# angela000/DQNFlappyBird

Hardware: AMD Instinct MI355X
Metric: env steps/sec (whole node) + DQN grad-steps/sec, 80x80x4 batch=32 (higher is better)
Workload: dtype f32

## Files before the change

dqnflappybird_amd/csrc/fb_qnet.hip:

```cpp
#include <math.h>
#include <stdlib.h>
#include "fb_common.h"

#ifndef FK_ABL
#define FK_ABL 0
#endif
#ifndef BW_ABL
#define BW_ABL 0
#endif

namespace {

typedef float f32x16 __attribute__((ext_vector_type(16)));

constexpr int OFF_W1 = 0, OFF_B1 = 8192, OFF_W2 = 8224, OFF_B2 = 40992, OFF_W3 = 41056, OFF_B3 = 77920,
              OFF_WF1 = 77984;
constexpr int CONV_PARAMS = OFF_WF1;
#include "fb_head.h"
#include "fb_sampler.h"
#include "fb_gather.h"
constexpr int MAXTB = 256;


struct Slice { const float *params; const uint8_t *states; int s_off, count; const uint16_t *w1s; int fshift; };
// ... 13 lines not shown
#pragma unroll
        for (int r = 0; r < 16; r++) { const int row = base + drow(r, lane); if (row < limit) body(r, row); }
    }
}

template <int NW, class F>
__device__ __forceinline__ void reduce_rows(const f32x16 &acc, float *red, int wave, int lane, int base, int limit, F body) {
    if (wave < NW) {
#pragma unroll
        for (int r = 0; r < 16; r++) red[(wave * 16 + r) * 64 + lane] = acc[r];
    }
    __syncthreads();
    if (wave >= 8) return;
    float v[2];
#pragma unroll
    for (int q = 0; q < 2; q++) {
        const int r = 2 * wave + q;
        v[q] = red[r * 64 + lane];
#pragma unroll
        for (int w = 1; w < NW; w++) v[q] += red[(w * 16 + r) * 64 + lane];
    }
    if (base + 32 <= limit) {
#pragma unroll
        for (int q = 0; q < 2; q++) body(v[q], 2 * wave + q, base + drow(2 * wave + q, lane));
    } else {
#pragma unroll
        for (int q = 0; q < 2; q++) { const int row = base + drow(2 * wave + q, lane); if (row < limit) body(v[q], 2 * wave + q, row); }
    }
}

__device__ __forceinline__ void keep(float &x) { asm volatile("" : "+v"(x)); }
__device__ __forceinline__ float rbf(float x, bool rb) { return rb ? (float)(__bf16)x : x; }
__device__ __forceinline__ void keep(int &x) { asm volatile("" : "+v"(x)); }

typedef __bf16 bf16x8 __attribute__((ext_vector_type(8)));

__device__ __forceinline__ uint32_t f32_to_bf16_rn(float x) {
    const uint32_t u = __float_as_uint(x);
    return (u + 0x7FFFu + ((u >> 16) & 1u)) >> 16;
}

__device__ __forceinline__ void split3(float x, uint32_t &hi, uint32_t &mid, uint32_t &lo) {
    hi = f32_to_bf16_rn(x);
    const float r1 = x - __uint_as_float(hi << 16);
    mid = f32_to_bf16_rn(r1);
    lo = f32_to_bf16_rn(r1 - __uint_as_float(mid << 16));
}

typedef __bf16 bf16x2 __attribute__((ext_vector_type(2)));
typedef float f32x2 __attribute__((ext_vector_type(2)));
__device__ __forceinline__ void split3x2(float x0, float x1, uint32_t &hi, uint32_t &mid, uint32_t &lo) {
    const f32x2 x = {x0, x1};
    const bf16x2 h = __builtin_convertvector(x, bf16x2);
    const f32x2 r1 = x - __builtin_convertvector(h, f32x2);
    const bf16x2 m = __builtin_convertvector(r1, bf16x2);
    const f32x2 r2 = r1 - __builtin_convertvector(m, f32x2);
    const bf16x2 l = __builtin_convertvector(r2, bf16x2);
    hi = __builtin_bit_cast(uint32_t, h); mid = __builtin_bit_cast(uint32_t, m); lo = __builtin_bit_cast(uint32_t, l);
}

typedef _Float16 f16x8 __attribute__((ext_vector_type(8)));
typedef _Float16 f16x2 __attribute__((ext_vector_type(2)));
constexpr float F16_LO_SCALE = 4096.f, F16_LO_UNSCALE = 1.f / 4096.f;
__device__ __forceinline__ void split2x2(float x0, float x1, uint32_t &hi, uint32_t &lo) {
    const f32x2 x = {x0, x1};
    const f16x2 h = __builtin_convertvector(x, f16x2);
// ... 1647 lines not shown
    float nq[AT], mean = 0.f;
#pragma unroll
    for (int a = 0; a < AT; a++) {
        const int o = (a < A ? a : 0) * N + il;
        nq[a] = draw(LQ.eout + o) * (ns[a] + H.sig[H.off.bq + o]);
        if (a < A) mean += nq[a];
    }
    if (DUEL) {
        mean /= (float)A;
        const float vn = draw(LV.eout + il) * (nv + H.sig[H.off.bv + il]);
#pragma unroll
        for (int a = 0; a < AT; a++) lg[a] += (vn + nq[a]) - mean;
    } else {
#pragma unroll
        for (int a = 0; a < AT; a++) lg[a] += nq[a];
    }
    float qv[AT];
    const float z = H.sup.vmin + (float)(on ? lane : 0) * H.sup.dz;
    c51_q<AT>(lg, on, z, qv);
    if (lane == 0 && live) {
#pragma unroll
        for (int a = 0; a < AT; a++) if (a < A) H.q[(size_t)smp * A + a] = qv[a];
        int best = 0;
#pragma unroll
        for (int a = 1; a < AT; a++) if (a < A && qv[a] > qv[best]) best = a;
        const fb_u4 o = fb_philox(H.seed_lo, H.seed_hi, (uint32_t)key, H.step_lo, H.stream, H.step_hi);
        const float u = (float)(o.x >> 8) * (1.0f / 16777216.0f);
        if (u <= H.epsilon) best = (int)(((unsigned long long)o.y * (unsigned)A) >> 32);
        H.actions[smp] = (uint8_t)best;
    }
}

typedef float f32x4 __attribute__((ext_vector_type(4)));
struct FkArgs { Slices sl; const float *h3; float *hf; float *qpart; int FC, A, dueling, stot; NetOff off; };
constexpr int FK_ROW = 204;

__global__ __launch_bounds__(512) void fc1_fk_kernel(FkArgs a) {
    __shared__ float ast[8 * 16 * FK_ROW];
    __shared__ float red[8 * 4 * 64];
    const Slice s = a.sl.s[blockIdx.z];
    const int M = s.count, m0 = blockIdx.x * 16, n0 = blockIdx.y * 16;
    if (m0 >= M) return;
    const int lane = threadIdx.x & 63, wave = threadIdx.x >> 6, r = lane & 15, g = lane >> 4;
    const int kw = wave * 200;
    const float *bcol = s.params + OFF_WF1 + (size_t)(kw + 50 * g) * a.FC + n0 + r;
    float bv[50];
#pragma unroll
    for (int t = 0; t < 50; t++) bv[t] = bcol[(size_t)(FK_ABL == 2 ? 0 : t) * a.FC];
    float hb = s.params[a.off.bf1 + n0 + r], hw[MAXA + 1];
#pragma unroll
    for (int c = 0; c < MAXA; c++) hw[c] = s.params[a.off.wq + (n0 + r) * a.A + (c < a.A ? c : 0)];
    hw[MAXA] = s.params[(a.dueling ? a.off.wv : a.off.bf1) + n0 + r];
    float *mine = ast + wave * 16 * FK_ROW;
    float4 st[13];
#pragma unroll
    for (int i = 0; i < 13; i++) {
        const int idx = lane + 64 * i, row = idx < 800 ? idx / 50 : 0, c4 = idx < 800 ? idx - row * 50 : 0;
        const int mr = m0 + row < M ? m0 + row : M - 1;
        st[i] = *reinterpret_cast<const float4 *>(a.h3 + (size_t)(s.s_off + mr) * 1600 + kw + 4 * (FK_ABL == 3 ? 0 : c4));
    }
#pragma unroll
    for (int i = 0; i < 13; i++) {
        const int idx = lane + 64 * i, row = idx / 50, c4 = idx - row * 50;
        if (idx < 800) *reinterpret_cast<float4 *>(mine + row * FK_ROW + 4 * c4) = st[i];
    }
    __builtin_amdgcn_wave_barrier();
    asm volatile("s_waitcnt lgkmcnt(0)" ::: "memory");
    const float *arow = mine + r * FK_ROW + 50 * g;
    f32x4 acc0 = {0.f, 0.f, 0.f, 0.f}, acc1 = {0.f, 0.f, 0.f, 0.f};
    float2 av[25];
#pragma unroll
    for (int t = 0; t < 25; t++) av[t] = *reinterpret_cast<const float2 *>(arow + 2 * t);
#pragma unroll
    for (int t = 0; t < 25; t++) { keep(av[t].x); keep(av[t].y); }
#pragma unroll
    for (int t = 0; t < (FK_ABL == 1 ? 1 : 25); t++) {
        acc0 = __builtin_amdgcn_mfma_f32_16x16x4f32(rbf(av[t].x, a.sl.rb), rbf(bv[2 * t], a.sl.rb), acc0, 0, 0, 0);
        acc1 = __builtin_amdgcn_mfma_f32_16x16x4f32(rbf(av[t].y, a.sl.rb), rbf(bv[2 * t + 1], a.sl.rb), acc1, 0, 0, 0);
    }
#pragma unroll
    for (int q = 0; q < 4; q++) red[(wave * 4 + q) * 64 + lane] = acc0[q] + acc1[q];
    __syncthreads();
    if (threadIdx.x >= 256) return;
    const int reg = threadIdx.x >> 6, row = 4 * g + reg, col = r, mr = m0 + row, unit = n0 + col;
    float v = red[reg * 64 + lane];
#pragma unroll
    for (int w = 1; w < 8; w++) v += red[(w * 4 + reg) * 64 + lane];
    const bool live = mr < M;
    const size_t srow = (size_t)s.s_off + (live ? mr : M - 1);
    if (live) a.hf[srow * a.FC + unit] = v;
    if (!a.qpart || FK_ABL == 4) return;
    const float h = fmaxf(v + hb, 0.f);
    const int qs = a.A + 1;
    float *qo = a.qpart + (srow * (size_t)gridDim.y + blockIdx.y) * qs;
#pragma unroll
    for (int c = 0; c <= MAXA; c++) {
        if (c < a.A || (c == a.A && a.dueling)) {
            float x = h * (c == a.A ? hw[MAXA] : hw[c]);
#pragma unroll
            for (int o = 8; o > 0; o >>= 1) x += __shfl_xor(x, o, 16);
            if (col == 0 && live) qo[c] = x;
        }
    }
}

struct Bw1Args {
    int algo, B, FC, A, dueling, stot, n_dx, rb;
    NetOff off;
    const float *params, *pnext, *ptarget;
    const float *hf, *qpart, *h3;
    const uint8_t *act; const float *rew; const uint8_t *term; const float *isw;
    double gamma;
    float *grad, *dh3, *loss, *abs_err, *y_out;
    AdamDev *adam; int tick;
    FbGate gate;
};
constexpr int BW_DX_ROW = 4;
constexpr int BW_DW_ROW = 36;

template <int AT, bool DX>
__device__ __forceinline__ void fc1_bwd2_body(const Bw1Args &L, float *smem) {
    const int tid = threadIdx.x, lane = tid & 63, wave = tid >> 6, B = L.B, FC = L.FC, A = AT == MAXA ? L.A : AT;
    const float *P = L.params;
    float (*dadv)[MAXA] = reinterpret_cast<float (*)[MAXA]>(smem);
    float *dv = smem + MAXTB * MAXA, *lterm = dv + MAXTB, *dadv2 = lterm + MAXTB, *big = dadv2 + 2 * MAXTB;
    const bool lead = blockIdx.x == 0;
    const bool dbl = L.algo == FB_ALGO_DOUBLE;
    const int qs = A + 1, ntile = FC >> 4;
    constexpr bool dx_role = DX;
    const int mt = dx_role ? blockIdx.x / 50 : 0, t2 = dx_role ? 0 : blockIdx.x - L.n_dx, nt = t2 / 7, kg = t2 - nt * 7;
    const int kt = dx_role ? blockIdx.x - mt * 50 : kg * 8 + wave;
    auto unit_params = [&](int n, float &bias, float (&wq)[AT], float &wv) {
        bias = P[L.off.bf1 + n];
        wv = P[(L.dueling ? L.off.wv : L.off.bf1) + n];
#pragma unroll
        for (int c = 0; c < AT; c++) wq[c] = P[L.off.wq + n * A + (c < A ? c : 0)];
    };
    float pre_hf[32], pre_bias, pre_wq[AT], pre_wv, pre_a[16];
    float4 pre_w[8];
    if constexpr (DX) {
        const int ch = FC < 512 ? FC : 512, n = tid < ch ? tid : 0;
#pragma unroll
        for (int q = 0; q < 32; q++) { const int bq_ = mt * 32 + q; pre_hf[q] = L.hf[(size_t)(bq_ < B ? bq_ : 0) * FC + n]; }
        unit_params(n, pre_bias, pre_wq, pre_wv);
        const int kh = ch / 16, nbeg = wave * (ch / 8) + (lane >> 5) * kh;
        const float *brun = P + OFF_WF1 + (size_t)(kt * 32 + (lane & 31)) * FC + nbeg;
#pragma unroll
        for (int q = 0; q < 8; q++) pre_w[q] = *reinterpret_cast<const float4 *>(brun + (4 * q < kh ? 4 * q : 0));
#pragma unroll
        for (int q = 0; q < 16; q++) pre_a[q] = 0.f;
#pragma unroll
        for (int q = 0; q < 2; q++) { const int mr = mt * 32 + drow(2 * (wave & 7) + q, lane); pre_a[q] = L.h3[(size_t)(mr < B ? mr : 0) * 1600 + kt * 32 + (lane & 31)]; }
    } else {
        const int c = tid & 31;
#pragma unroll
        for (int q = 0; q < 2; q++) { const int b = (tid >> 5) + 16 * q; pre_hf[q] = L.hf[(size_t)(b < B ? b : 0) * FC + nt * 32 + c]; }
#pragma unroll
        for (int q = 2; q < 32; q++) pre_hf[q] = 0.f;
        unit_params(nt * 32 + c, pre_bias, pre_wq, pre_wv);
        const int ktc = kt < 50 ? kt : 0;
#pragma unroll
        for (int t = 0; t < 16; t++) { const int b = 2 * t + (lane >> 5); pre_a[t] = L.h3[(size_t)(b < B ? b : 0) * 1600 + ktc * 32 + (lane & 31)]; }
#pragma unroll
        for (int q = 0; q < 8; q++) pre_w[q] = make_float4(0.f, 0.f, 0.f, 0.f);
    }
    float bqs[AT], bqn[AT], bq3[AT];
#pragma unroll
    for (int c = 0; c < AT; c++) { const int cc = c < A ? c : 0; bqs[c] = L.params[L.off.bq + cc]; bqn[c] = L.pnext[L.off.bq + cc]; bq3[c] = L.ptarget[L.off.bq + cc]; }
    const int bvo = L.dueling ? L.off.bv : L.off.bq;
    float bvs = L.params[bvo], bvn = L.pnext[bvo], bv3 = L.ptarget[bvo];
    for (int b0 = 0; b0 < (BW_ABL == 1 ? 0 : B); b0 += 32) {
        const int b = b0 + (tid >> 4), j = tid & 15, bc = b < B ? b : 0;
        float rf = L.rew[bc], isw = L.isw ? L.isw[bc] : 1.f;
        int termb = L.term[bc], a_b = L.act[bc];
        float x0[2][AT + 1], x1[2][AT + 1], x2[2][AT + 1];
#pragma unroll
        for (int u = 0; u < 2; u++) {
            const int tile = j + 16 * u, tc = tile < ntile ? tile : 0;
            const float *q0 = L.qpart + ((size_t)bc * ntile + tc) * qs;
            const size_t rs = (size_t)ntile * qs;
#pragma unroll
            for (int c = 0; c <= AT; c++) {
                const int cc = c < qs ? c : 0;
                x0[u][c] = q0[cc]; x1[u][c] = q0[(size_t)B * rs + cc]; x2[u][c] = q0[(size_t)(dbl ? 2 * B : 0) * rs + cc];
            }
        }
        keep(rf); keep(isw); keep(termb); keep(a_b);
        float qsv[AT + 1], qnv[AT + 1], q3v[AT + 1];
#pragma unroll
        for (int c = 0; c <= AT; c++) {
            keep(x0[0][c]); keep(x1[0][c]); keep(x2[0][c]); keep(x0[1][c]); keep(x1[1][c]); keep(x2[1][c]);
            const bool on = c < A || (c == A && L.dueling), on0 = on && j < ntile, on1 = on && j + 16 < ntile;
            qsv[c] = (on0 ? x0[0][c] : 0.f) + (on1 ? x0[1][c] : 0.f);
            qnv[c] = (on0 ? x1[0][c] : 0.f) + (on1 ? x1[1][c] : 0.f);
            q3v[c] = (on0 ? x2[0][c] : 0.f) + (on1 ? x2[1][c] : 0.f);
        }
        for (int tile = j + 32; tile < ntile; tile += 16) {
// ... 39 lines not shown
        if (L.algo != FB_ALGO_PER) isw = 1.f;
        const double rr = rf == 0.1f ? 0.1 : (double)rf;
        const double yd = termb ? rr : rr + L.gamma * (double)sel;
        const float y = (float)yd;
        float qe = qsv[0];
#pragma unroll
        for (int c = 1; c < AT; c++) qe = c == a_b ? qsv[c] : qe;
        const float d = y - qe;
        const float scale = L.algo == FB_ALGO_DQN ? 2.f : 2.f / (float)B;
        const float gq = -scale * isw * d;
        const bool pg = L.algo == FB_ALGO_PG;
        float pgp[AT], pgl;
        {
            float mx = qsv[0], se = 0.f;
#pragma unroll
            for (int c = 1; c < AT; c++) mx = c < A ? fmaxf(mx, qsv[c]) : mx;
#pragma unroll
            for (int c = 0; c < AT; c++) { pgp[c] = c < A ? expf(qsv[c] - mx) : 0.f; se += pgp[c]; }
#pragma unroll
            for (int c = 0; c < AT; c++) pgp[c] /= se;
            pgl = logf(se) - (qe - mx);
        }
        const float pgw = rf / (float)L.gamma;
        if (j == 0 && b < B) {
            lterm[b] = pg ? pgl * pgw : isw * d * d;
            if (lead && L.abs_err) L.abs_err[b] = fabsf(d);
            if (lead && L.y_out) L.y_out[b] = y;
            dv[b] = L.dueling && !pg ? gq : 0.f;
#pragma unroll
            for (int c = 0; c < AT; c++) dadv[b][c] = pg ? (pgp[c] - (c == a_b ? 1.f : 0.f)) * pgw : (c == a_b ? gq : 0.f) - (L.dueling ? gq / (float)A : 0.f);
            if (AT == 2) { dadv2[2 * b] = dadv[b][0]; dadv2[2 * b + 1] = dadv[b][1]; }
        }
    }
#pragma unroll
    for (int q = 0; q < 32; q++) keep(pre_hf[q]);
#pragma unroll
    for (int q = 0; q < 16; q++) keep(pre_a[q]);
#pragma unroll
    for (int q = 0; q < 8; q++) { keep(pre_w[q].x); keep(pre_w[q].y); keep(pre_w[q].z); keep(pre_w[q].w); }
    __syncthreads();
    if (lead && tid == 0) {
        float sum = 0.f;
        for (int b = 0; b < B; b++) sum += lterm[b];
        *L.loss = L.algo == FB_ALGO_DQN || L.algo == FB_ALGO_PG ? sum : sum / (float)B;
        if (L.tick && L.adam->ticks == L.adam->applies) {
            AdamDev &ad = *L.adam;
            ad.alpha = ad.lr * sqrtf(1.f - ad.b2pow) / (1.f - ad.b1pow);
            ad.b1pow *= ad.b1; ad.b2pow *= ad.b2;
            ad.ticks += 1;
        }
    }
    if (lead && tid >= 64 && tid < 64 + A) { const int c = tid - 64; float sum = 0.f; for (int b = 0; b < B; b++) sum += dadv[b][c]; L.grad[L.off.bq + c] = sum; }
    if (lead && tid == 128 && L.dueling) { float sum = 0.f; for (int b = 0; b < B; b++) sum += dv[b]; L.grad[L.off.bv] = sum; }
    auto dhf_of = [&](int b, float hfv, float bias, const float (&wq)[AT], float wv, float &hout) {
        const float v = hfv + bias;
        float d = L.dueling ? dv[b] * wv : 0.f;
#pragma unroll
        for (int c = 0; c < AT; c++) if (c < A) d = fmaf(dadv[b][c], wq[c], d);
        hout = fmaxf(v, 0.f);
        return v > 0.f ? d : 0.f;
    };
    const int hl = lane >> 5, i = lane & 31, jj = lane & 31;
    if constexpr (DX) {
        const int RS = 512 + BW_DX_ROW;
        float *dh = big, *red = big + 32 * RS;
        f32x16 acc = {0};
        for (int nc = 0; nc < FC; nc += 512) {
            const int ch = FC - nc < 512 ? FC - nc : 512;
            if (nc) {
                __syncthreads();
                const int n = nc + (tid < ch ? tid : 0);
#pragma unroll
                for (int q = 0; q < 32; q++) { const int bq_ = mt * 32 + q; pre_hf[q] = L.hf[(size_t)(bq_ < B ? bq_ : 0) * FC + n]; }
                unit_params(n, pre_bias, pre_wq, pre_wv);
                const int kh = ch / 16, nbeg = wave * (ch / 8) + hl * kh;
                const float *brun = P + OFF_WF1 + (size_t)(kt * 32 + jj) * FC + nc + nbeg;
#pragma unroll
                for (int q = 0; q < 8; q++) pre_w[q] = *reinterpret_cast<const float4 *>(brun + (4 * q < kh ? 4 * q : 0));
            }
            if (tid < ch && BW_ABL != 2) {
                if (AT == 2 && !L.dueling) {
                    float4 da[16];
#pragma unroll
                    for (int q = 0; q < 16; q++) da[q] = *reinterpret_cast<const float4 *>(dadv2 + 2 * (mt * 32 + 2 * q < MAXTB - 1 ? mt * 32 + 2 * q : 0));
                    float o[32];
#pragma unroll
                    for (int q = 0; q < 16; q++) {
                        const float v0 = pre_hf[2 * q] + pre_bias, v1 = pre_hf[2 * q + 1] + pre_bias;
                        const float d0 = fmaf(da[q].y, pre_wq[1], fmaf(da[q].x, pre_wq[0], 0.f)), d1 = fmaf(da[q].w, pre_wq[1], fmaf(da[q].z, pre_wq[0], 0.f));
                        o[2 * q] = (v0 > 0.f && mt * 32 + 2 * q < B) ? d0 : 0.f;
                        o[2 * q + 1] = (v1 > 0.f && mt * 32 + 2 * q + 1 < B) ? d1 : 0.f;
                    }
#pragma unroll
                    for (int q = 0; q < 32; q++) dh[q * RS + tid] = o[q];
                } else {
#pragma unroll
                    for (int q = 0; q < 32; q++) {
                        float hv;
                        dh[q * RS + tid] = mt * 32 + q < B ? dhf_of(mt * 32 + q, pre_hf[q], pre_bias, pre_wq, pre_wv, hv) : 0.f;
                    }
                }
            }
            __syncthreads();
            const int kh = ch / 16, nbeg = wave * (ch / 8) + hl * kh;
            const float *arun = dh + i * RS + nbeg;
            float4 xa[8];
#pragma unroll
            for (int q = 0; q < 8; q++) xa[q] = *reinterpret_cast<const float4 *>(arun + (4 * q < kh ? 4 * q : 0));
#pragma unroll
            for (int q = 0; q < 8; q++) { keep(xa[q].x); keep(xa[q].y); keep(xa[q].z); keep(xa[q].w); }
#pragma unroll
            for (int q = 0; q < 8; q++) {
                if (4 * q < kh && BW_ABL != 3) {
                    const float4 x = xa[q], w = pre_w[q];
                    const bool rb = L.rb;
                    acc = mfma(rbf(x.x, rb), rbf(w.x, rb), acc); acc = mfma(rbf(x.y, rb), rbf(w.y, rb), acc);
                    acc = mfma(rbf(x.z, rb), rbf(w.z, rb), acc); acc = mfma(rbf(x.w, rb), rbf(w.w, rb), acc);
                }
            }
        }
        reduce_rows<8>(acc, red, wave, lane, mt * 32, B, [&](float v, int r, int mr) {
            const size_t o = (size_t)mr * 1600 + kt * 32 + jj;
            L.dh3[o] = BW_ABL == 4 ? v : (((r & 1) ? pre_a[1] : pre_a[0]) > 0.f ? v : 0.f);
        });
        return;
    }
    if (BW_ABL == 5) return;
    float *dh = big, *hh = big + MAXTB * BW_DW_ROW;
    {
        const int c = tid & 31;
#pragma unroll
        for (int q = 0; q < 2; q++) {
            const int b = (tid >> 5) + 16 * q;
// ... 1078 lines not shown
                (i >= off.bf1 && i < off.bf1 + FC) || (i >= off.bq && i < off.bq + A) || (dueling && i == off.bv);
    if (bias) { p[i] = 0.01f; return; }
    for (uint32_t ctr = 0;; ctr++) {
        const fb_u4 r = fb_philox(seed_lo, seed_hi, (uint32_t)i, ctr, FB_STREAM_INIT, 0u);
        const float u1 = ((r.x >> 8) + 1) * (1.0f / 16777216.0f), u2 = (r.y >> 8) * (1.0f / 16777216.0f);
        const float z = sqrtf(-2.f * logf(u1)) * cosf(6.28318530717958647692f * u2);
        if (fabsf(z) <= 2.f) { p[i] = 0.01f * z; return; }
    }
}

}

#ifndef FB_ADAM_GRID
#define FB_ADAM_GRID 1024
#endif
constexpr int ADAM_GRID = FB_ADAM_GRID;

struct fb_qnet {
    int arch, FC, A, max_batch;
    long long n;
    NetOff off;
    float *params[2], *adam_m, *adam_v, *grad, *slabs;
    float *slabs1;
    uint16_t *w1s[2];
    uint4 *wsp[2];
    uint16_t *zeros;
    uint16_t *a1s, *a3s;
    int nsplit;
    int nsplit_train;
    bool adam_ticked;
    AdamDev *adam;
    float *p1, *h2, *h3, *hf, *q;
    float *qpart;
    unsigned long long *ring_fo;
    hipEvent_t grad_ev;
    hipEvent_t grad_ev_recorded;
    uint8_t *amax;
    float *dhf, *dh3, *dh2, *dp1;
    float *gmax;
    int zmax;
    float *hf_act, *hp_act;
    FbSplitCtx *split;
    C51Sup sup;
    float kappa;
    float *c51_dl, *c51_xs, *c51_lt;
    NetOff hoff;
    float *heff[2];
    bool noisy;
    long long ntot;
    NoisyNet nnet;
    float *mst[2], *nz[2];
    int act_noise;
    float *nz_zero, *ht;
    uint4 *wsig;
    uint16_t *a3n;
    int *sig_seen;
    bool split_adam_pending;
};

static NetOff make_off(int FC, int A, int dueling) {
    NetOff o;
    o.bf1 = OFF_WF1 + 1600 * FC;
    int p = o.bf1 + FC;
    if (dueling) { o.wv = p; o.bv = p + FC; p = o.bv + 1; } else { o.wv = 0; o.bv = 0; }
    o.wq = p; o.bq = p + FC * A; o.n = o.bq + A;
    return o;
// ... 118 lines not shown
    h->hoff = is_c51d(h) ? make_off(fc_width, n_actions * sup.N, 0) : h->off;
    h->n = h->off.n;
    h->noisy = sigma0 >= 0.f;
    h->ntot = h->noisy ? 2 * h->n - OFF_WF1 : h->n;
    if (h->noisy) h->nnet = make_noisy(h->off, arch, fc_width, n_actions, sup.N, sigma0);
    h->zmax = 64;
    const size_t S = (size_t)3 * max_batch, nb = sizeof(float) * (size_t)h->n, nbt = sizeof(float) * (size_t)h->ntot;
    hipError_t e = hipSuccess;
    auto alloc = [&](void **p, size_t bytes) { if (e == hipSuccess) e = hipMalloc(p, bytes); if (e == hipSuccess) e = hipMemset(*p, 0, bytes); };
    alloc((void **)&h->params[0], nb); alloc((void **)&h->params[1], nb);
    alloc((void **)&h->adam_m, nbt); alloc((void **)&h->adam_v, nbt); alloc((void **)&h->grad, nbt);
    if (h->noisy) for (int w = 0; w < 2; w++) { alloc((void **)&h->mst[w], nbt); alloc((void **)&h->nz[w], sizeof(float) * (size_t)h->nnet.nz); }
    if (h->noisy) {
        alloc((void **)&h->nz_zero, sizeof(float) * (size_t)h->nnet.nz);
        alloc((void **)&h->wsig, sizeof(uint4) * (size_t)wsp_w3t(fc_width));
        alloc((void **)&h->a3n, S * 1600 * 6 + 256);
        alloc((void **)&h->ht, S * fc_width * 4 * FC1_SP_KS);
        alloc((void **)&h->sig_seen, sizeof(int));
        if (e == hipSuccess) e = hipMemset(h->sig_seen, 0xff, sizeof(int));
    }
    alloc((void **)&h->slabs, sizeof(float) * (size_t)h->zmax * CONV_PARAMS);
    if (2 * max_batch > h->zmax) alloc((void **)&h->slabs1, sizeof(float) * (size_t)2 * (max_batch < MAXTB ? max_batch : MAXTB) * CONV1_PARAMS);
    alloc((void **)&h->adam, sizeof(AdamDev));
    alloc((void **)&h->w1s[0], 3 * 8192 * 2); alloc((void **)&h->w1s[1], 3 * 8192 * 2);
    const size_t wsp_bytes = (size_t)wsp_total(fc_width) * sizeof(uint4);
    alloc((void **)&h->wsp[0], wsp_bytes); alloc((void **)&h->wsp[1], wsp_bytes);
    h->nsplit = 3; h->nsplit_train = 3;
    alloc((void **)&h->zeros, 256);
    alloc((void **)&h->a1s, S * 3200 * 6); alloc((void **)&h->a3s, S * 1600 * 6 + 256);
    alloc((void **)&h->p1, S * 3200 * 4); alloc((void **)&h->amax, S * 3200);
    alloc((void **)&h->h2, S * 1600 * 4); alloc((void **)&h->h3, S * 1600 * 4);
    alloc((void **)&h->hf, S * fc_width * 4 * FC1_KS); alloc((void **)&h->q, S * MAXA * 4);
    alloc((void **)&h->qpart, (size_t)(fc_width / 16) * S * (MAXA + 1) * 4);
    alloc((void **)&h->ring_fo, (size_t)max_batch * 4 * sizeof(unsigned long long));
    const size_t Bm = max_batch;
    alloc((void **)&h->dhf, Bm * fc_width * 4); alloc((void **)&h->dh3, Bm * 1600 * 4);
    alloc((void **)&h->dh2, Bm * 1600 * 4); alloc((void **)&h->dp1, Bm * 3200 * 4);
    alloc((void **)&h->gmax, (size_t)(fc_width / 16) * 4);
    alloc((void **)&h->hf_act, S * fc_width * 4 * FC1_SP_KS); alloc((void **)&h->hp_act, sizeof(float) * (size_t)(h->n - h->off.bf1));
    if (sup.N) { alloc((void **)&h->c51_dl, Bm * 64 * 4); alloc((void **)&h->c51_xs, Bm * fc_width * 4); alloc((void **)&h->c51_lt, Bm * 4); }
    if (is_c51d(h)) for (int w = 0; w < 2; w++) alloc((void **)&h->heff[w], sizeof(float) * (size_t)(h->hoff.n - h->off.bf1));
    if (e != hipSuccess) {
        fb_set_error(e == hipErrorOutOfMemory ? FB_ERR_NOMEM : FB_ERR_HIP, "fb_qnet_create: %s", hipGetErrorString(e));
        fb_qnet_destroy(h);
        return e == hipErrorOutOfMemory ? FB_ERR_NOMEM : FB_ERR_HIP;
    }
    *out = h;
    {
        AdamDev a; memset(&a, 0, sizeof(a));
        a.pver[0] = a.pver[1] = 1;
        if (hipMemcpy(h->adam, &a, sizeof(a), hipMemcpyHostToDevice) != hipSuccess) { fb_qnet_destroy(h); *out = nullptr; return fb_set_error(FB_ERR_HIP, "fb_qnet_create: hipMemcpy failed"); }
    }
    return fb_qnet_set_hparams(h, 1e-6f, 0.9f, 0.999f, 1e-8f);
}

extern "C" int fb_qnet_destroy(fb_qnet_t h) {
    if (!h) return FB_OK;
    void *ptrs[] = {h->zeros, h->wsp[0], h->wsp[1], h->a1s, h->a3s, h->w1s[0], h->w1s[1], h->params[0], h->params[1], h->adam_m, h->adam_v, h->grad, h->slabs, h->slabs1, h->adam, h->p1, h->amax, h->h2,
                    h->h3, h->hf, h->q, h->qpart, h->dhf, h->dh3, h->dh2, h->dp1, h->ring_fo, h->gmax, h->hf_act, h->hp_act,
                    h->c51_dl, h->c51_xs, h->c51_lt, h->heff[0], h->heff[1], h->mst[0], h->mst[1], h->nz[0], h->nz[1],
                    h->nz_zero, h->wsig, h->a3n, h->ht, h->sig_seen};
    if (h->split) {
        FbSplitCtx *c = h->split;
        if (c->tstream) { (void)hipStreamSynchronize(c->tstream); (void)hipStreamDestroy(c->tstream); }
        if (c->f) (void)hipFree(c->f);
        delete c;
    }
    for (void *p : ptrs) if (p) (void)hipFree(p);
    delete h;
    return FB_OK;
}

__global__ void flag_wait_kernel(const unsigned long long *flag, unsigned long long v, unsigned *timeouts) { if (threadIdx.x == 0) fb_flag_wait(flag, v, timeouts); }
__global__ void flag_set_kernel(unsigned long long *flag, unsigned long long v) { fb_flag_store(flag, v); }

FbSplitCtx *fb_qnet_split_ctx(fb_qnet_t h) {
    if (!h) return nullptr;
    if (h->split) return h->split->tstream ? h->split : nullptr;
    FbSplitCtx *c = new FbSplitCtx();
    memset(c, 0, sizeof(*c));
    h->split = c;
    int lo = 0, hi = 0;
    bool ok = hipMalloc((void **)&c->f, sizeof(FbSplitFlags)) == hipSuccess && hipMemset(c->f, 0, sizeof(FbSplitFlags)) == hipSuccess;
    hipStream_t ts = nullptr;
    ok = ok && hipDeviceGetStreamPriorityRange(&lo, &hi) == hipSuccess && hipStreamCreateWithPriority(&ts, hipStreamNonBlocking, lo) == hipSuccess;
    if (!ok) { (void)hipGetLastError(); return nullptr; }
    c->tstream = ts;
    return c;
}

int fb_split_probe(FbSplitCtx *c, void *stream) {
    if (!c || !c->tstream) return 0;
// ... 251 lines not shown
            const int rows_f = af.M;
            const dim3 gc((rows + 4) / 5), gf(((rows_f + 127) / 128) * (h->FC / 64) * FC1_SP_KS);
            if (fused && p.split && only < 0 && gc.x > 256 && gc.x % 256 != 0) { c23.round_flag = &p.split->f->last_round; c23.round_val = p.split->seq; c23.round_blk = (int)(gc.x / 256) * 256; }
            if (nsp == 3) {
                if (fused) { FB_K(K_CONV2) hipLaunchKernelGGL((conv23_sp_kernel<3, 5, true>), gc, dim3(512), 0, st, c23); }
                else if (!trunk) { FB_K(K_CONV2) hipLaunchKernelGGL(conv23_sp_kernel<3>, gc, dim3(512), 0, st, c23); }
                FB_K(K_FC1) hipLaunchKernelGGL(fc1_sp_kernel<3>, gf, dim3(256), 0, st, af);
            } else {
                if (fused) { FB_K(K_CONV2) hipLaunchKernelGGL((conv23_sp_kernel<1, 5, true>), gc, dim3(512), 0, st, c23); }
                else if (!trunk) { FB_K(K_CONV2) hipLaunchKernelGGL(conv23_sp_kernel<1>, gc, dim3(512), 0, st, c23); }
                FB_K(K_FC1) hipLaunchKernelGGL(fc1_sp_kernel<1>, gf, dim3(256), 0, st, af);
            }
            if (fused && (only < 0 || only == K_FC1) && (long long)af.hp_n > (long long)gf.x * 256) {
                const size_t done = (size_t)gf.x * 256;
                FB_CHECK_HIP(hipMemcpyAsync(h->hp_act + done, af.hp_src + done, sizeof(float) * ((size_t)af.hp_n - done), hipMemcpyDeviceToDevice, st));
            }
            z0 = z1;
        }
    }
    if (!sp && !trunk) FB_K(K_CONV1) {
        const dim3 g1((t1 + 3) / 4, 1, p.ns);
        if (p.nib) hipLaunchKernelGGL(conv1_pool_kernel<true>, g1, dim3(256), 0, st, p.sl, h->p1, h->amax, job);
        else hipLaunchKernelGGL(conv1_pool_kernel<false>, g1, dim3(256), 0, st, p.sl, h->p1, h->amax, job);
    }
    if (!sp && !trunk) FB_K(K_CONV2) {
        if (nsp == 3) hipLaunchKernelGGL((conv23_t_kernel<3, false>), dim3(maxc, p.ns), dim3(512), 0, st, c23t);
        else hipLaunchKernelGGL((conv23_t_kernel<1, false>), dim3(maxc, p.ns), dim3(512), 0, st, c23t);
    }
    const bool fk = !sp && !big;
    const bool c51 = h->sup.N > 0;
    if (fk) FB_K(K_FC1) {
        FkArgs fa;
        fa.sl = p.sl; fa.h3 = h->h3; fa.hf = h->hf; fa.qpart = p.train && !c51 ? h->qpart : nullptr; fa.FC = h->FC; fa.A = h->A;
        fa.dueling = h->arch == FB_ARCH_DUELING; fa.stot = stot; fa.off = h->off;
        hipLaunchKernelGGL(fc1_fk_kernel, dim3((maxc + 15) / 16, h->FC / 16, p.ns), dim3(512), 0, st, fa);
    }
    if (c51 && !p.train && !p.no_head) FB_K(K_HEAD) {
        C51HeadArgs H;
        H.sl = p.sl; H.nslices = p.ns; H.params = nullptr;
        for (int z = 0; z < p.ns; z++) H.sl.s[z].params = head_base(h, p.sl.s[z].params);
        C51Core &C = H.c;
        C.hf = acting_fused ? h->hf_act : h->hf; C.stot = stot; C.nks = sp ? FC1_SP_KS : 1; C.q = h->q; C.probs = p.probs; C.FC = h->FC; C.A = h->A;
        C.off = h->hoff; C.sup = h->sup; C.actions = p.actions; C.epsilon = p.epsilon;
        C.seed_lo = (uint32_t)p.seed; C.seed_hi = (uint32_t)(p.seed >> 32);
        C.step_lo = (uint32_t)p.step; C.step_hi = (uint32_t)(p.step >> 32);
        C.key_of = nullptr; C.stream = FB_STREAM_EPS;
        if (p.head_rider) {
            memset(p.head_rider, 0, sizeof(*p.head_rider));
            p.head_rider->c.hf = C.hf; p.head_rider->c.stot = stot; p.head_rider->c.nks = C.nks;
            p.head_rider->params = acting_fused ? h->hp_act - h->off.bf1 : H.sl.s[0].params;
        } else if (is_qr(h) && h->A == 2) hipLaunchKernelGGL(qr_head_kernel<2>, dim3((total + 3) / 4), dim3(256), 0, st, H);
        else if (is_qr(h)) hipLaunchKernelGGL(qr_head_kernel<MAXA>, dim3((total + 3) / 4), dim3(256), 0, st, H);
        else if (h->A == 2) hipLaunchKernelGGL(c51_head_kernel<2>, dim3((total + 3) / 4), dim3(256), 0, st, H);
        else hipLaunchKernelGGL(c51_head_kernel<MAXA>, dim3((total + 3) / 4), dim3(256), 0, st, H);
    }
    if (!c51 && !(fk && p.train)) FB_K(K_HEAD) {
        HeadArgs H;
        H.sl = p.sl; H.nslices = p.ns;
        HeadCore &C = H.c;
        C.hf = acting_fused ? h->hf_act : h->hf; C.stot = stot; C.nks = sp ? FC1_SP_KS : 1; C.q = h->q; C.FC = h->FC; C.A = h->A;
        C.dueling = h->arch == FB_ARCH_DUELING; C.off = h->off; C.actions = p.actions; C.epsilon = p.epsilon;
        C.seed_lo = (uint32_t)p.seed; C.seed_hi = (uint32_t)(p.seed >> 32);
        C.step_lo = (uint32_t)p.step; C.step_hi = (uint32_t)(p.step >> 32);
        if (p.head_rider) { p.head_rider->c = C; p.head_rider->params = acting_fused ? h->hp_act - h->off.bf1 : p.sl.s[0].params; p.head_rider->on = 1; p.head_rider->on_arrival = nullptr; p.head_rider->arrival_val = 0; }
        else hipLaunchKernelGGL(head_kernel, dim3((total + 3) / 4), dim3(256), 0, st, H);
    }
    if (p.train) {
// ... 25 lines not shown
            L.algo = is_double_c51(p.algo) ? FB_ALGO_C51_DOUBLE : FB_ALGO_C51;
            L.B = B; L.FC = FC; L.A = h->A; L.nks = fk ? 1 : FC1_SP_KS; L.stot = stot; L.off = h->hoff; L.sup = h->sup;
            L.p_on = head_base(h, h->params[0]); L.p_next = head_base(h, p.sl.s[1].params);
            L.p_tgt = head_base(h, p.ns > 2 ? p.sl.s[2].params : p.sl.s[1].params);
            L.hf = h->hf; L.act = p.a; L.rew = p.r; L.term = p.t; L.gamma = p.gamma;
            L.dl = h->c51_dl; L.xs = h->c51_xs; L.lterm = h->c51_lt; L.dhf = h->dhf;
            L.isw = pw ? p.isw : nullptr; L.abs_err = pw ? p.abs_err : nullptr;
            if (pw && h->A == 2) hipLaunchKernelGGL((c51_loss_kernel<2, true>), dim3((B + 3) / 4), dim3(256), 0, st, L);
            else if (pw) hipLaunchKernelGGL((c51_loss_kernel<MAXA, true>), dim3((B + 3) / 4), dim3(256), 0, st, L);
            else if (h->A == 2) hipLaunchKernelGGL(c51_loss_kernel<2>, dim3((B + 3) / 4), dim3(256), 0, st, L);
            else hipLaunchKernelGGL(c51_loss_kernel<MAXA>, dim3((B + 3) / 4), dim3(256), 0, st, L);
            const C51GradArgs gA{B, FC, h->A, h->sup.N, h->off, h->c51_dl, h->c51_xs, h->c51_lt, h->dhf, p.a, G, p.loss, h->gmax, h->adam, p.tick};
            if (is_c51d(h)) hipLaunchKernelGGL(c51d_grad_kernel, dim3(FC / 16), dim3(256), 0, st, gA);
            else hipLaunchKernelGGL(c51_grad_kernel, dim3(FC / 16), dim3(256), 0, st, gA);
        }
        if (!fk && !c51) FB_K(K_LOSS) {
            LossArgs L;
            L.algo = p.algo; L.B = B; L.FC = FC; L.A = h->A; L.dueling = h->arch == FB_ARCH_DUELING; L.off = h->off;
            L.params = h->params[0]; L.q = h->q; L.hf = h->hf; L.stot = stot; L.nks = FC1_SP_KS; L.act = p.a; L.rew = p.r; L.term = p.t; L.isw = p.isw;
            L.gamma = p.gamma; L.grad = G; L.dhf = h->dhf; L.loss = p.loss; L.abs_err = p.abs_err; L.y_out = p.y; L.gmax = h->gmax;
            if (p.tick) h->adam_ticked = !p.apply_adam;
            L.adam = h->adam; L.tick = p.tick;
            hipLaunchKernelGGL(loss_head_kernel, dim3(FC / 16), dim3(256), 0, st, L);
        }
        int z3 = (B * 25 + 255) / 256, z1 = (B * 400 + 255) / 256;
        if (z3 > h->zmax) z3 = h->zmax;
        if (z1 > h->zmax) z1 = h->zmax;
        const size_t ss = CONV_PARAMS;
        const int ndx1 = ((B + 31) / 32) * 50;
        if (fk && !c51) { FB_K(K_FC1_BWD) {
            Bw1Args L;
            L.algo = p.algo; L.B = B; L.FC = FC; L.A = h->A; L.dueling = h->arch == FB_ARCH_DUELING; L.stot = stot; L.n_dx = ndx1; L.off = h->off;
            L.params = h->params[0]; L.pnext = p.sl.s[1].params; L.ptarget = p.ns > 2 ? p.sl.s[2].params : p.sl.s[1].params;
            L.hf = h->hf; L.qpart = h->qpart; L.h3 = h->h3; L.act = p.a; L.rew = p.r; L.term = p.t; L.isw = p.isw; L.gamma = p.gamma;
            L.grad = G; L.dh3 = h->dh3; L.loss = p.loss; L.abs_err = p.abs_err; L.y_out = p.y;
            if (p.tick) h->adam_ticked = !p.apply_adam;
            L.adam = h->adam; L.tick = p.tick; L.rb = rbt;
            L.gate = FbGate{nullptr, 0, nullptr};
            if (p.split && only < 0) L.gate = FbGate{&p.split->f->trunk_done, p.split->seq, &p.split->f->timeouts[2]};
            hipLaunchKernelGGL(fc1_bwd2_kernel, dim3(ndx1 + (FC / 32) * 7 + (L.gate.flag ? 1 : 0)), dim3(512), 0, st, L);
        } } else FB_K(K_FC1_BWD) {
            const int ndx = ((B + 31) / 32) * 50, ntile = ndx + 50 * (FC / 32);
            const dim3 gb(ntile);
            const bool std_shape = FC == 512 && B == 256;
            if (h->nsplit_train == 3) {
                if (std_shape) hipLaunchKernelGGL((fc1_bwd_big_kernel<3, 4, 2>), gb, dim3(512), 0, st, ndx, h->params[0], h->h3, h->dhf, h->dh3, G, B, FC, (const float *)h->gmax, &h->adam->ovf);
                else hipLaunchKernelGGL((fc1_bwd_big_kernel<3, 0, 0>), gb, dim3(512), 0, st, ndx, h->params[0], h->h3, h->dhf, h->dh3, G, B, FC, (const float *)h->gmax, &h->adam->ovf);
            } else {
                if (std_shape) hipLaunchKernelGGL((fc1_bwd_big_kernel<1, 4, 2>), gb, dim3(512), 0, st, ndx, h->params[0], h->h3, h->dhf, h->dh3, G, B, FC, (const float *)h->gmax, &h->adam->ovf);
                else hipLaunchKernelGGL((fc1_bwd_big_kernel<1, 0, 0>), gb, dim3(512), 0, st, ndx, h->params[0], h->h3, h->dhf, h->dh3, G, B, FC, (const float *)h->gmax, &h->adam->ovf);
            }
        }
        if (!p.apply_adam && only < 0) {
            h->grad_ev_recorded = nullptr;
            if (h->grad_ev) { FB_CHECK_HIP(hipEventRecord(h->grad_ev, st)); h->grad_ev_recorded = h->grad_ev; }
        }
        const int span0 = OFF_WF1 / 4, span1 = p.apply_adam ? (OFF_WF1 + 1600 * FC) / 4 : span0;
        const AdamSpan span{master(h, 0), h->adam_m, h->adam_v, G, h->adam, span0, span1};
        FbGate gate_fc1{nullptr, 0, nullptr};
        if (p.split && only < 0) gate_fc1 = FbGate{&p.split->f->fc1_done, p.split->seq, &p.split->f->timeouts[3]};
        FbSampleRider srider;
        memset(&srider, 0, sizeof(srider));
        if (p.sample_rider) srider = *p.sample_rider;
        {
            const bool fold1 = 2 * B > h->zmax;
            const int fold = (2 * B + h->zmax - 1) / h->zmax;
            z1 = fold1 ? (2 * B + fold - 1) / fold : 2 * B;
// ... 478 lines not shown
```

Measured before the change: 11.24 million.

## Store FC1 ReLU activity bitmask in forward and use it in backward dx

The fused FC1 forward kernel now writes a 16-bit ballot mask per row and 16-unit tile that records which units have a positive pre-activation. The FC1 backward dx blocks load this compact mask instead of 32 full float hf values per unit, and use it to gate the ReLU derivative. This cuts global memory traffic and register pressure in the backward prefetch. The cost is an extra mask buffer and a ballot plus store in the forward pass. Correctness depends on the mask row layout and the mt*32 indexing lining up with the training slice offsets.

```diff
diff --git a/dqnflappybird_amd/csrc/fb_qnet.hip b/dqnflappybird_amd/csrc/fb_qnet.hip
--- a/dqnflappybird_amd/csrc/fb_qnet.hip
+++ b/dqnflappybird_amd/csrc/fb_qnet.hip
@@ -69,6 +69,7 @@
 __device__ __forceinline__ void keep(float &x) { asm volatile("" : "+v"(x)); }
 __device__ __forceinline__ float rbf(float x, bool rb) { return rb ? (float)(__bf16)x : x; }
 __device__ __forceinline__ void keep(int &x) { asm volatile("" : "+v"(x)); }
+__device__ __forceinline__ void keep(unsigned &x) { asm volatile("" : "+v"(x)); }
 
 typedef __bf16 bf16x8 __attribute__((ext_vector_type(8)));
 
@@ -1782,7 +1783,7 @@
 }
 
 typedef float f32x4 __attribute__((ext_vector_type(4)));
-struct FkArgs { Slices sl; const float *h3; float *hf; float *qpart; int FC, A, dueling, stot; NetOff off; };
+struct FkArgs { Slices sl; const float *h3; float *hf; float *qpart; uint16_t *fmask; int FC, A, dueling, stot, fmask_rs; NetOff off; };
 constexpr int FK_ROW = 204;
 
 __global__ __launch_bounds__(512) void fc1_fk_kernel(FkArgs a) {
@@ -1840,6 +1841,8 @@
     const size_t srow = (size_t)s.s_off + (live ? mr : M - 1);
     if (live) a.hf[srow * a.FC + unit] = v;
     if (!a.qpart || FK_ABL == 4) return;
+    const unsigned long long on = __ballot(live && v + hb > 0.f);
+    if (col == 0 && live) a.fmask[(size_t)blockIdx.y * a.fmask_rs + srow] = (uint16_t)(on >> (16 * g));
     const float h = fmaxf(v + hb, 0.f);
     const int qs = a.A + 1;
     float *qo = a.qpart + (srow * (size_t)gridDim.y + blockIdx.y) * qs;
@@ -1859,6 +1862,7 @@
     NetOff off;
     const float *params, *pnext, *ptarget;
     const float *hf, *qpart, *h3;
+    const uint16_t *fmask; int fmask_rs;
     const uint8_t *act; const float *rew; const uint8_t *term; const float *isw;
     double gamma;
     float *grad, *dh3, *loss, *abs_err, *y_out;
@@ -1888,10 +1892,15 @@
     };
     float pre_hf[32], pre_bias, pre_wq[AT], pre_wv, pre_a[16];
     float4 pre_w[8];
+    uint4 pre_m[4];
+    auto load_mask = [&](int n) {
+        const uint4 *mp = reinterpret_cast<const uint4 *>(L.fmask + (size_t)(n >> 4) * L.fmask_rs + mt * 32);
+#pragma unroll
+        for (int q = 0; q < 4; q++) pre_m[q] = mp[q];
+    };
     if constexpr (DX) {
         const int ch = FC < 512 ? FC : 512, n = tid < ch ? tid : 0;
-#pragma unroll
-        for (int q = 0; q < 32; q++) { const int bq_ = mt * 32 + q; pre_hf[q] = L.hf[(size_t)(bq_ < B ? bq_ : 0) * FC + n]; }
+        load_mask(n);
         unit_params(n, pre_bias, pre_wq, pre_wv);
         const int kh = ch / 16, nbeg = wave * (ch / 8) + (lane >> 5) * kh;
         const float *brun = P + OFF_WF1 + (size_t)(kt * 32 + (lane & 31)) * FC + nbeg;
@@ -1913,6 +1922,8 @@
         for (int t = 0; t < 16; t++) { const int b = 2 * t + (lane >> 5); pre_a[t] = L.h3[(size_t)(b < B ? b : 0) * 1600 + ktc * 32 + (lane & 31)]; }
 #pragma unroll
         for (int q = 0; q < 8; q++) pre_w[q] = make_float4(0.f, 0.f, 0.f, 0.f);
+#pragma unroll
+        for (int q = 0; q < 4; q++) pre_m[q] = make_uint4(0u, 0u, 0u, 0u);
     }
     float bqs[AT], bqn[AT], bq3[AT];
 #pragma unroll
@@ -2018,8 +2029,13 @@
             if (AT == 2) { dadv2[2 * b] = dadv[b][0]; dadv2[2 * b + 1] = dadv[b][1]; }
         }
     }
-#pragma unroll
-    for (int q = 0; q < 32; q++) keep(pre_hf[q]);
+    if constexpr (DX) {
+#pragma unroll
+        for (int q = 0; q < 4; q++) { keep(pre_m[q].x); keep(pre_m[q].y); keep(pre_m[q].z); keep(pre_m[q].w); }
+    } else {
+#pragma unroll
+        for (int q = 0; q < 32; q++) keep(pre_hf[q]);
+    }
 #pragma unroll
     for (int q = 0; q < 16; q++) keep(pre_a[q]);
 #pragma unroll
@@ -2038,11 +2054,15 @@
     }
     if (lead && tid >= 64 && tid < 64 + A) { const int c = tid - 64; float sum = 0.f; for (int b = 0; b < B; b++) sum += dadv[b][c]; L.grad[L.off.bq + c] = sum; }
     if (lead && tid == 128 && L.dueling) { float sum = 0.f; for (int b = 0; b < B; b++) sum += dv[b]; L.grad[L.off.bv] = sum; }
+    auto dhf_sum = [&](int b, const float (&wq)[AT], float wv) {
+        float d = L.dueling ? dv[b] * wv : 0.f;
+#pragma unroll
+        for (int c = 0; c < AT; c++) if (c < A) d = fmaf(dadv[b][c], wq[c], d);
+        return d;
+    };
     auto dhf_of = [&](int b, float hfv, float bias, const float (&wq)[AT], float wv, float &hout) {
         const float v = hfv + bias;
-        float d = L.dueling ? dv[b] * wv : 0.f;
-#pragma unroll
-        for (int c = 0; c < AT; c++) if (c < A) d = fmaf(dadv[b][c], wq[c], d);
+        const float d = dhf_sum(b, wq, wv);
         hout = fmaxf(v, 0.f);
         return v > 0.f ? d : 0.f;
     };
@@ -2056,8 +2076,7 @@
             if (nc) {
                 __syncthreads();
                 const int n = nc + (tid < ch ? tid : 0);
-#pragma unroll
-                for (int q = 0; q < 32; q++) { const int bq_ = mt * 32 + q; pre_hf[q] = L.hf[(size_t)(bq_ < B ? bq_ : 0) * FC + n]; }
+                load_mask(n);
                 unit_params(n, pre_bias, pre_wq, pre_wv);
                 const int kh = ch / 16, nbeg = wave * (ch / 8) + hl * kh;
                 const float *brun = P + OFF_WF1 + (size_t)(kt * 32 + jj) * FC + nc + nbeg;
@@ -2065,6 +2084,13 @@
                 for (int q = 0; q < 8; q++) pre_w[q] = *reinterpret_cast<const float4 *>(brun + (4 * q < kh ? 4 * q : 0));
             }
             if (tid < ch && BW_ABL != 2) {
+                const int bit = (nc + tid) & 15;
+                auto on = [&](int q) {
+                    const uint4 m = pre_m[q >> 3];
+                    const int w = (q >> 1) & 3;
+                    const uint32_t v = w == 0 ? m.x : w == 1 ? m.y : w == 2 ? m.z : m.w;
+                    return ((v >> (16 * (q & 1) + bit)) & 1u) != 0u;
+                };
                 if (AT == 2 && !L.dueling) {
                     float4 da[16];
 #pragma unroll
@@ -2072,19 +2098,15 @@
                     float o[32];
 #pragma unroll
                     for (int q = 0; q < 16; q++) {
-                        const float v0 = pre_hf[2 * q] + pre_bias, v1 = pre_hf[2 * q + 1] + pre_bias;
                         const float d0 = fmaf(da[q].y, pre_wq[1], fmaf(da[q].x, pre_wq[0], 0.f)), d1 = fmaf(da[q].w, pre_wq[1], fmaf(da[q].z, pre_wq[0], 0.f));
-                        o[2 * q] = (v0 > 0.f && mt * 32 + 2 * q < B) ? d0 : 0.f;
-                        o[2 * q + 1] = (v1 > 0.f && mt * 32 + 2 * q + 1 < B) ? d1 : 0.f;
+                        o[2 * q] = (on(2 * q) && mt * 32 + 2 * q < B) ? d0 : 0.f;
+                        o[2 * q + 1] = (on(2 * q + 1) && mt * 32 + 2 * q + 1 < B) ? d1 : 0.f;
                     }
 #pragma unroll
                     for (int q = 0; q < 32; q++) dh[q * RS + tid] = o[q];
                 } else {
 #pragma unroll
-                    for (int q = 0; q < 32; q++) {
-                        float hv;
-                        dh[q * RS + tid] = mt * 32 + q < B ? dhf_of(mt * 32 + q, pre_hf[q], pre_bias, pre_wq, pre_wv, hv) : 0.f;
-                    }
+                    for (int q = 0; q < 32; q++) dh[q * RS + tid] = mt * 32 + q < B && on(q) ? dhf_sum(mt * 32 + q, pre_wq, pre_wv) : 0.f;
                 }
             }
             __syncthreads();
@@ -3229,6 +3251,7 @@
     AdamDev *adam;
     float *p1, *h2, *h3, *hf, *q;
     float *qpart;
+    uint16_t *fmask; int fmask_rs;
     unsigned long long *ring_fo;
     hipEvent_t grad_ev;
     hipEvent_t grad_ev_recorded;
@@ -3413,6 +3436,8 @@
     alloc((void **)&h->h2, S * 1600 * 4); alloc((void **)&h->h3, S * 1600 * 4);
     alloc((void **)&h->hf, S * fc_width * 4 * FC1_KS); alloc((void **)&h->q, S * MAXA * 4);
     alloc((void **)&h->qpart, (size_t)(fc_width / 16) * S * (MAXA + 1) * 4);
+    h->fmask_rs = (int)((S + 31) / 32 * 32);
+    alloc((void **)&h->fmask, (size_t)(fc_width / 16) * h->fmask_rs * sizeof(uint16_t));
     alloc((void **)&h->ring_fo, (size_t)max_batch * 4 * sizeof(unsigned long long));
     const size_t Bm = max_batch;
     alloc((void **)&h->dhf, Bm * fc_width * 4); alloc((void **)&h->dh3, Bm * 1600 * 4);
@@ -3438,7 +3463,7 @@
 extern "C" int fb_qnet_destroy(fb_qnet_t h) {
     if (!h) return FB_OK;
     void *ptrs[] = {h->zeros, h->wsp[0], h->wsp[1], h->a1s, h->a3s, h->w1s[0], h->w1s[1], h->params[0], h->params[1], h->adam_m, h->adam_v, h->grad, h->slabs, h->slabs1, h->adam, h->p1, h->amax, h->h2,
-                    h->h3, h->hf, h->q, h->qpart, h->dhf, h->dh3, h->dh2, h->dp1, h->ring_fo, h->gmax, h->hf_act, h->hp_act,
+                    h->h3, h->hf, h->q, h->qpart, h->fmask, h->dhf, h->dh3, h->dh2, h->dp1, h->ring_fo, h->gmax, h->hf_act, h->hp_act,
                     h->c51_dl, h->c51_xs, h->c51_lt, h->heff[0], h->heff[1], h->mst[0], h->mst[1], h->nz[0], h->nz[1],
                     h->nz_zero, h->wsig, h->a3n, h->ht, h->sig_seen};
     if (h->split) {
@@ -3756,7 +3781,7 @@
     if (fk) FB_K(K_FC1) {
         FkArgs fa;
         fa.sl = p.sl; fa.h3 = h->h3; fa.hf = h->hf; fa.qpart = p.train && !c51 ? h->qpart : nullptr; fa.FC = h->FC; fa.A = h->A;
-        fa.dueling = h->arch == FB_ARCH_DUELING; fa.stot = stot; fa.off = h->off;
+        fa.dueling = h->arch == FB_ARCH_DUELING; fa.stot = stot; fa.off = h->off; fa.fmask = h->fmask; fa.fmask_rs = h->fmask_rs;
         hipLaunchKernelGGL(fc1_fk_kernel, dim3((maxc + 15) / 16, h->FC / 16, p.ns), dim3(512), 0, st, fa);
     }
     if (c51 && !p.train && !p.no_head) FB_K(K_HEAD) {
@@ -3848,7 +3873,7 @@
             Bw1Args L;
             L.algo = p.algo; L.B = B; L.FC = FC; L.A = h->A; L.dueling = h->arch == FB_ARCH_DUELING; L.stot = stot; L.n_dx = ndx1; L.off = h->off;
             L.params = h->params[0]; L.pnext = p.sl.s[1].params; L.ptarget = p.ns > 2 ? p.sl.s[2].params : p.sl.s[1].params;
-            L.hf = h->hf; L.qpart = h->qpart; L.h3 = h->h3; L.act = p.a; L.rew = p.r; L.term = p.t; L.isw = p.isw; L.gamma = p.gamma;
+            L.hf = h->hf; L.qpart = h->qpart; L.fmask = h->fmask; L.fmask_rs = h->fmask_rs; L.h3 = h->h3; L.act = p.a; L.rew = p.r; L.term = p.t; L.isw = p.isw; L.gamma = p.gamma;
             L.grad = G; L.dh3 = h->dh3; L.loss = p.loss; L.abs_err = p.abs_err; L.y_out = p.y;
             if (p.tick) h->adam_ticked = !p.apply_adam;
             L.adam = h->adam; L.tick = p.tick; L.rb = rbt;
```

Result: no change. 11.34 million, median of 6 (+0.8%).
